# retab-dev/k-LLMs

Hardware: NVIDIA H100
Metric: consensus records/sec at n=16 (1M x 32-field); achieved HBM GB/s vs peak (higher is better)
Workload: dtype i32 codes / f64 values

## Files before the change

include/kllms_b200.h:

```cpp
#ifndef KLLMS_B200_H
#define KLLMS_B200_H

#include <stdint.h>

#ifdef __cplusplus
extern "C" {
#endif

#define KC_VERSION 200
#define KC_MAX_CANDIDATES 64

#define KC_OK 0
#define KC_EINVAL (-1)
#define KC_ECUDA (-2)
#define KC_ENODEV (-3)
#define KC_ENOMEM (-4)

#define KC_CODE_NONE (-1)
#define KC_CODE_ABSENT (-2)

#define KC_F64_NONE_BITS 0x7FF8C0DE00000000ULL
#define KC_F64_ABSENT_BITS 0x7FF8C0DF00000000ULL

#define KC_META_IDX(m) ((uint32_t)(m) & 0x3Fu)
// ... 106 lines not shown
int kc_align_json_batch(const char *const *texts, const int64_t *lens, int64_t n_records, int32_t n, double min_support_ratio, int device,
                        int32_t threads, char **out_texts, int32_t *out_status, int64_t *out_counts);
int kc_debug_similarity_json(const char *a, const char *b, double *out);
int kc_debug_alignsim(const char *const *texts, int32_t T, double *out);
int kc_debug_alignsim_nodes(const char *const *texts, const int32_t *node_len, int32_t n_nodes, int32_t lanes, int device, double *out);
int kc_debug_lsap(int32_t nr, int32_t nc, const double *cost, int32_t *row_ind, int32_t *col_ind);

int kc_consolidate_json(const char *const *texts, const int64_t *lens, int64_t n_records, int32_t n, double rel_eps,
                        double abs_eps, int device, int32_t threads, char **out_content, char **out_likelihoods,
                        uint8_t *out_status);
void kc_free_strings(char **arr, int64_t count);

#define KC_JSON_DEVICE_ONLY 1u
#define KC_JSON_NUMERIC_MEDOID 2u
#define KC_JSON_KEY_UNION 4u
#define KC_JSON_LISTS 8u
#define KC_JSON_UNICODE 16u
typedef struct kc_json_result kc_json_result;
typedef struct {
    int64_t n_records, n_device, n_host, n_python;
    int64_t input_bytes, output_bytes;
    int32_t chunks, streams;
    double h2d_ms, plan_ms , kernel_ms , emit_ms , d2h_ms;
    double device_path_wall_ms, host_path_wall_ms, wall_ms;
} kc_json_stats;
int kc_consolidate_json_packed(const char *h_text, const int64_t *h_off, int64_t n_records, int32_t n, double rel_eps, double abs_eps,
                               int device, int32_t threads, uint32_t flags, kc_json_result **out);
int kc_consolidate_json_packed_weighted(const char *h_text, const int64_t *h_off, const float *h_seq_logprob, int64_t n_records, int32_t n,
                                        double rel_eps, double abs_eps, int device, int32_t threads, uint32_t flags, kc_json_result **out);
int kc_json_result_view(kc_json_result *res, const char **text, const int64_t **content_off, const int64_t **content_len,
                        const int64_t **likelihoods_off, const int64_t **likelihoods_len, const uint8_t **status, const uint8_t **why,
                        kc_json_stats *stats);
void kc_json_result_free(kc_json_result *res);

typedef struct kc_debug_jsongpu kc_debug_jsongpu;
int kc_debug_jsongpu_plan(const char *h_text, const int64_t *h_off, int64_t n_records, int32_t n, kc_debug_jsongpu **out);
int kc_debug_jsongpu_plan_flags(const char *h_text, const int64_t *h_off, int64_t n_records, int32_t n, uint32_t flags,
                                kc_debug_jsongpu **out);
int kc_debug_jsongpu_inputs(const kc_debug_jsongpu *h, const int8_t **vote_cells, int64_t *n_vote_groups, const double **num_cells,
                            int64_t *n_num_groups, const uint8_t **status);
int kc_debug_jsongpu_emit(kc_debug_jsongpu *h, const uint32_t *vote_meta, const double *num_value, const uint32_t *num_meta,
                          const char **content, const int64_t **content_off, const char **likelihoods, const int64_t **likelihoods_off);
int kc_debug_jsongpu_group_records(const kc_debug_jsongpu *h, const int32_t **group_record);
int kc_debug_jsongpu_emit_weighted(kc_debug_jsongpu *h, const uint32_t *vote_meta, const float *vote_weight, const double *num_value,
                                   const uint32_t *num_meta, const char **content, const int64_t **content_off, const char **likelihoods,
                                   const int64_t **likelihoods_off);
int kc_debug_jsongpu_medoid_inputs(const kc_debug_jsongpu *h, const uint8_t **chars, const int32_t **str_off, const int32_t **grp_off,
                                   int64_t *n_groups);
int kc_debug_jsongpu_set_medoid(kc_debug_jsongpu *h, const int32_t *medoid_idx, const double *medoid_avg);
int kc_debug_jsongpu_set_numeric_medoid(kc_debug_jsongpu *h, const int32_t *best, const double *best_avg);
void kc_debug_jsongpu_free(kc_debug_jsongpu *h);
int kc_debug_parse_doubles(const char *text, const int64_t *off, int64_t count, double *out, uint8_t *ok);
int kc_debug_float_reprs(const double *xs, int64_t count, char *out , int32_t *lens);
int kc_debug_parse_doubles_device(const char *text, const int64_t *off, int64_t count, double *out, uint8_t *ok, int device);
int kc_debug_float_reprs_device(const double *xs, int64_t count, char *out , int32_t *lens, int device);
int kc_debug_round5(const double *xs, int64_t count, double *out);
int kc_debug_s32_texts(uint64_t seed, int64_t n_records, int32_t n, int32_t threads, char *out, int64_t cap, int64_t *off);

int32_t kc_levenshtein(const char *a, int32_t alen, const char *b, int32_t blen);

void *kc_host_alloc(uint64_t bytes);
void kc_host_free(void *p);

#ifdef __cplusplus
}
#endif
// ... 2 lines not shown
```

k_llms_b200/_native.py:

```python
from __future__ import annotations

import ctypes
import os
from typing import Optional, Tuple

_HERE = os.path.dirname(os.path.abspath(__file__))
LIB_PATH = os.environ.get("KLLMS_B200_LIB") or os.path.join(_HERE, "libkllms_b200.so")

KC_OK, KC_EINVAL, KC_ECUDA, KC_ENODEV, KC_ENOMEM = 0, -1, -2, -3, -4
MAX_CANDIDATES = 64
CODE_NONE, CODE_ABSENT = -1, -2
F64_NONE_BITS = 0x7FF8C0DE00000000
F64_ABSENT_BITS = 0x7FF8C0DF00000000
FLAG_HAS_VALUE, FLAG_SINGLE, FLAG_TIE, FLAG_NO_FINITE = 1, 2, 4, 8
OUT_LOCAL, OUT_MULTIMEM, OUT_PEERS = 0, 1, 2

_vp, _i32, _i64, _u32, _u64, _f64 = ctypes.c_void_p, ctypes.c_int32, ctypes.c_int64, ctypes.c_uint32, ctypes.c_uint64, ctypes.c_double
_int, _str, _pp = ctypes.c_int, ctypes.c_char_p, ctypes.POINTER(ctypes.c_void_p)
_CONSENSUS_HOST = [_vp, _i32, _vp, _vp, _i32, _i64, _i32, _f64, _f64, _vp, _vp, _vp, _vp, _int, _vp]

_SIGNATURES = {
    "kc_version": (_int, []),
    "kc_last_error": (_str, []),
    "kc_device_count": (_int, []),
# ... 2 lines not shown
    "kc_vote_i32": (_int, [_vp, _i64, _i32, _vp, _i32, _vp, _vp, _vp]),
    "kc_vote_i32_ex": (_int, [_vp, _i64, _i32, _vp, _i32, _vp, _vp, _u32, _vp]),
    "kc_vote_i32_peers": (_int, [_vp, _i64, _i32, _vp, _i32, _vp, _vp, _i32, _vp, _vp]),
    "kc_vote_i32_peers_packed": (_int, [_vp, _i64, _i32, _vp, _i32, _vp, _vp, _vp, _i32, _vp, _vp, _vp]),
    "kc_vote_i32_wire": (_int, [_vp, _i64, _i32, _vp, _i32, _vp, _vp, _vp, _i32, _i32, _vp, _vp, _vp]),
    "kc_vote_i8": (_int, [_vp, _i64, _i32, _vp, _i32, _vp, _vp, _vp]),
    "kc_numeric_f64": (_int, [_vp, _i64, _i32, _f64, _f64, _vp, _vp, _vp]),
    "kc_numeric_f64_ex": (_int, [_vp, _i64, _i32, _f64, _f64, _vp, _vp, _u32, _vp]),
    "kc_numeric_f64_peers": (_int, [_vp, _i64, _i32, _f64, _f64, _vp, _vp, _i32, _vp, _vp]),
    "kc_push_results": (_int, [_vp, _vp, _i64, _vp, _vp, _i64, _vp, _vp, _vp, _i32, _i32, _vp, _vp, _i32, _vp]),
    "kc_confidence_f64": (_int, [_vp, _i64, _i32, _vp, _vp, _vp]),
    "kc_logprob_sum_f32": (_int, [_vp, _vp, _i64, _vp, _vp]),
    "kc_weighted_vote_i32": (_int, [_vp, _vp, _i64, _i32, _i32, _vp, _vp, _vp, _vp, _vp]),
    "kc_weighted_vote_groups_i8": (_int, [_vp, _i64, _i32, _vp, _vp, _i64, _vp, _vp, _vp, _vp]),
    "kc_consensus_host": (_int, _CONSENSUS_HOST),
    "kc_consensus_host_i8": (_int, _CONSENSUS_HOST),
    "kc_host_alloc": (_vp, [_u64]),
    "kc_host_free": (None, [_vp]),
    "kc_medoid_str": (_int, [_vp, _vp, _vp, _i64, _i32, _vp, _vp, _vp]),
    "kc_medoid_str_method": (_int, [_vp, _vp, _vp, _i64, _i32, _i32, _vp, _vp, _vp]),
    "kc_medoid_str_host": (_int, [_vp, _i64, _vp, _vp, _i64, _i32, _vp, _vp, _int]),
    "kc_numeric_medoid_f64": (_int, [_vp, _i64, _i32, _vp, _vp, _vp]),
    "kc_levenshtein": (_int, [_str, _i32, _str, _i32]),
    "kc_consolidate_json": (_int, [_vp, _vp, _i64, _i32, _f64, _f64, _int, _i32, _vp, _vp, _vp]),
    "kc_free_strings": (None, [_vp, _i64]),
    "kc_align_json": (_int, [ctypes.POINTER(_str), _vp, _i32, _f64, ctypes.POINTER(_str)]),
    "kc_align_json_batch": (_int, [_vp, _vp, _i64, _i32, _f64, _int, _i32, _vp, _vp, _vp]),
    "kc_json_plan": (_int, [_vp, _vp, _i64, _i32, _i32, _pp]),
    "kc_json_inputs": (_int, [_vp] * 10),
    "kc_json_emit": (_int, [_vp] * 9),
    "kc_json_free": (None, [_vp]),
    "kc_consolidate_json_packed": (_int, [_vp, _vp, _i64, _i32, _f64, _f64, _int, _i32, _u32, _pp]),
    "kc_consolidate_json_packed_weighted": (_int, [_vp, _vp, _vp, _i64, _i32, _f64, _f64, _int, _i32, _u32, _pp]),
    "kc_json_result_view": (_int, [_vp] + [_pp] * 7 + [_vp]),
    "kc_json_result_free": (None, [_vp]),
    "kc_debug_similarity_json": (_int, [_str, _str, ctypes.POINTER(_f64)]),
    "kc_debug_lsap": (_int, [_i32, _i32, _vp, _vp, _vp]),
    "kc_debug_alignsim": (_int, [_vp, _i32, _vp]),
    "kc_debug_alignsim_nodes": (_int, [_vp, _vp, _i32, _i32, _int, _vp]),
    "kc_debug_jsongpu_plan": (_int, [_vp, _vp, _i64, _i32, _pp]),
    "kc_debug_jsongpu_plan_flags": (_int, [_vp, _vp, _i64, _i32, _u32, _pp]),
    "kc_debug_jsongpu_inputs": (_int, [_vp] * 6),
    "kc_debug_jsongpu_emit": (_int, [_vp, _vp, _vp, _vp] + [_pp] * 4),
    "kc_debug_jsongpu_group_records": (_int, [_vp, _pp]),
    "kc_debug_jsongpu_emit_weighted": (_int, [_vp, _vp, _vp, _vp, _vp] + [_pp] * 4),
    "kc_debug_jsongpu_medoid_inputs": (_int, [_vp] + [_pp] * 3 + [ctypes.POINTER(_i64)]),
    "kc_debug_jsongpu_set_medoid": (_int, [_vp, _vp, _vp]),
    "kc_debug_jsongpu_set_numeric_medoid": (_int, [_vp, _vp, _vp]),
    "kc_debug_jsongpu_free": (None, [_vp]),
    "kc_debug_parse_doubles": (_int, [_vp, _vp, _i64, _vp, _vp]),
    "kc_debug_float_reprs": (_int, [_vp, _i64, _vp, _vp]),
    "kc_debug_parse_doubles_device": (_int, [_vp, _vp, _i64, _vp, _vp, _int]),
    "kc_debug_float_reprs_device": (_int, [_vp, _i64, _vp, _vp, _int]),
    "kc_debug_round5": (_int, [_vp, _i64, _vp]),
    "kc_debug_s32_texts": (_int, [_u64, _i64, _i32, _i32, _vp, _i64, _vp]),
}
EXPORTS = tuple(_SIGNATURES)


class NativeError(RuntimeError):
    def __init__(self, code: int, what: str):
        super().__init__(f"libkllms_b200: {what} (code {code})")
        self.code = code


_lib: Optional[ctypes.CDLL] = None
# ... 420 lines not shown
```

k_llms_b200/csrc/kc_jsongpu.cu:

```cuda
#include <cuda_runtime.h>

#include <algorithm>
#include <atomic>
#include <chrono>
#include <cstdio>
#include <cstdlib>
#include <cstring>
#include <mutex>
#include <string>
#include <thread>
#include <type_traits>
#include <vector>

#include <cub/device/device_scan.cuh>
#include <nvtx3/nvToolsExt.h>

#include "../../include/kllms_b200.h"
#include "kc_internal.h"
#include "kc_jsongpu.cuh"

namespace {

using kc::js::Chunk;
using kc::js::Tok;

#define R_(call)                              \
    do {                                      \
        if (const int rc_ = (call)) return rc_; \
    } while (0)

enum Stage { RECORDS, SLOTS, UNION, SCRATCH, CSR, OFF };
struct Units {
    size_t R, B, T = 0, P = 0, S = 0;
};
template <class Alloc>
int chunk_arrays(const Alloc &alloc, Chunk &ch, Stage stage, const Units &u, size_t keep, bool vrec) {
    const size_t n = (size_t)ch.n;
    int k = 0;
    auto a = [&](Stage st, auto *&ptr, size_t count, size_t per, size_t plus, int fill, bool on_device) {
        const int i = k++;
        return st == stage ? alloc(i, ptr, count * per + plus, keep * per, fill, on_device) : KC_OK;
    };
    R_(a(RECORDS, ch.fcount, u.R, 1, 1, 0, true));
    R_(a(RECORDS, ch.slot, u.R, 1, 1, 0, false));
// ... 7 lines not shown
    R_(a(RECORDS, ch.mcount, u.R, 1, 1, 0, true));
    R_(a(RECORDS, ch.scount, u.R, 1, 1, 0, true));
    R_(a(RECORDS, ch.ccount, u.R, 1, 1, 0, true));
    R_(a(RECORDS, ch.len_c, u.R, 1, 1, 0, true));
    R_(a(RECORDS, ch.len_l, u.R, 1, 1, 0, true));
    R_(a(SLOTS, ch.toks, u.T, n, 1, 0, false));
    R_(a(SLOTS, ch.fdesc, u.T, 1, 1, 0, false));
    R_(a(SLOTS, ch.gpos, u.T, 1, 1, 0, false));
    R_(a(SLOTS, ch.piece_c, u.T, 1, 1, 0, false));
    R_(a(SLOTS, ch.piece_l, u.T, 1, 1, 0, false));
    R_(a(SLOTS, ch.vcells, u.T, n, 16, 0xFF, true));
    R_(a(SLOTS, ch.xcells, u.T, n, 2, 0, true));
    R_(a(vrec ? SLOTS : OFF, ch.vrec, u.T, 1, 1, 0xFF, false));
    R_(a(UNION, ch.ucand, u.P, n, 0, 0, false));
    R_(a(UNION, ch.ubase, u.P, 1, 0, 0, false));
    R_(a(UNION, ch.usize, u.P, 1, 0, 0, false));
    R_(a(SCRATCH, ch.utok, u.S, 1, 0, 0, false));
    R_(a(SCRATCH, ch.unode, u.S, 1, 0, 0, false));
    R_(a(SCRATCH, ch.umap, u.S, 1, 0, 0xFF, false));
    R_(a(CSR, ch.mchars, u.B, 1, 16, 0, false));
    R_(a(CSR, ch.mstr_off, u.T, n, 2, 0, false));
    R_(a(CSR, ch.mgrp_off, u.T, 1, 2, 0, false));
    return KC_OK;
}

void set_flags(Chunk &ch, uint32_t flags, uint8_t lists, int32_t aligned0) {
    ch.xmedoid = (flags & KC_JSON_NUMERIC_MEDOID) != 0;
    ch.key_union = (flags & KC_JSON_KEY_UNION) != 0;
    ch.unicode = (flags & KC_JSON_UNICODE) != 0;
    ch.lists = lists;
    ch.aligned0 = aligned0;
}

struct Worker {
    int device = -1;
    cudaStream_t stream = nullptr;
    cudaEvent_t ev[7] = {};
    kc::GrowBuf<kc::Mem::Device> text, off, counters, win, vmeta, xvalue, xmeta, out_c, out_l, scan_tmp, midx, mavg, seq, vweight;
    std::vector<kc::GrowBuf<kc::Mem::Device>> arrays;
    kc::GrowBuf<kc::Mem::Pinned> h_small;
    kc::GrowBuf<kc::Mem::Pinned> h_scan;
    bool busy = false;
    int init(int dev) {
        if (device == dev) return KC_OK;
        KC_CUDA_I(cudaStreamCreateWithFlags(&stream, cudaStreamNonBlocking));
        for (auto &e : ev) KC_CUDA_I(cudaEventCreate(&e));
        device = dev;
        return KC_OK;
    }
};

std::mutex g_pool_mu;
std::vector<Worker *> g_workers;

Worker *acquire_worker(int device) {
    std::lock_guard<std::mutex> lock(g_pool_mu);
    for (Worker *w : g_workers)
        if (!w->busy && w->device == device) {
            w->busy = true;
            return w;
        }
    Worker *w = new Worker;
    w->busy = true;
    g_workers.push_back(w);
    return w;
}
void release_worker(Worker *w) {
    std::lock_guard<std::mutex> lock(g_pool_mu);
    w->busy = false;
}

struct PinnedBlob {
    char *p = nullptr;
    size_t cap = 0;
};
std::vector<PinnedBlob> g_blob_pool;

PinnedBlob acquire_blob(size_t need) {
    {
// ... 48 lines not shown
        ptr = w.arrays[(size_t)k].as<E>();
        if (on_device) KC_CUDA_I(cudaMemsetAsync(ptr + keep_len, fill, (len - keep_len) * sizeof(E), w.stream));
        return KC_OK;
    };
    R_(chunk_arrays(dev, ch, stage, u, keep, weighted));
    if (stage != SLOTS) return KC_OK;
    const size_t T1 = std::max<size_t>(u.T, 1);
    R_(w.win.reserve(T1 * 4));
    R_(w.vmeta.reserve(T1 * 4));
    R_(w.xvalue.reserve(T1 * 8));
    R_(w.xmeta.reserve(T1 * 4));
    ch.vmeta = w.vmeta.as<uint32_t>();
    ch.xvalue = w.xvalue.as<double>();
    ch.xmeta = w.xmeta.as<uint32_t>();
    ch.xbest = w.xmeta.as<int32_t>();
    ch.xavg = w.xvalue.as<double>();
    if (weighted) {
        R_(w.vweight.reserve(T1 * 4));
        ch.vweight = w.vweight.as<float>();
    }
    return KC_OK;
}

template <typename T>
void exclusive_scan(T *v, size_t len) {
    T acc = 0;
    for (size_t i = 0; i < len; ++i) {
        const T c = v[i];
        v[i] = acc;
        acc += c;
    }
}

}

struct kc_json_result {
    int64_t R = 0;
    PinnedBlob blob;
    std::atomic<int64_t> used{0};
    std::vector<int64_t> c_off, c_len, l_off, l_len;
    std::vector<uint8_t> status, why;
    std::string heap;
    kc_json_stats stats{};
};

namespace {

struct ChunkStage {
    float h2d = 0, plan = 0, kernels = 0, emit = 0, d2h = 0;
};

int union_round(Worker &w, Chunk &ch, Units &u, int team, int grid, bool weighted, unsigned long long *h_cnt) {
    cudaStream_t s = w.stream;
    const int32_t P = (int32_t)u.P;
    R_(device_arrays(w, ch, UNION, u, 0, weighted));
    ch.uslot = (uint32_t)u.T;
    kc::js::union_count_kernel<<<grid, 128, 0, s>>>(ch, team, P);
    KC_CUDA_I(cudaGetLastError());
    KC_CUDA_I(cudaMemcpyAsync(h_cnt, ch.counters, 48, cudaMemcpyDeviceToHost, s));
    KC_CUDA_I(cudaStreamSynchronize(s));
    u.S = std::max<size_t>(h_cnt[4], 1);
    if (u.S >= ((size_t)1 << 32)) return kc_fail(KC_EINVAL, "kc_consolidate_json_packed: %zu union scratch entries in one chunk", u.S);
    R_(device_arrays(w, ch, SCRATCH, u, 0, weighted));
    kc::js::union_build_kernel<<<grid, 128, 0, s>>>(ch, team, P);
    KC_CUDA_I(cudaGetLastError());
    KC_CUDA_I(cudaMemcpyAsync(h_cnt, ch.counters, 48, cudaMemcpyDeviceToHost, s));
    KC_CUDA_I(cudaStreamSynchronize(s));
    if (const size_t U = h_cnt[5]) {
        const size_t keep = u.T;
        u.T += U;
        if (u.T >= ((size_t)1 << 32)) return kc_fail(KC_EINVAL, "kc_consolidate_json_packed: %zu field slots in one chunk", u.T);
        R_(device_arrays(w, ch, SLOTS, u, keep, weighted));
    }
    kc::js::union_plan_kernel<<<grid, 128, 0, s>>>(ch, team, P);
    KC_CUDA_I(cudaGetLastError());
    KC_CUDA_I(cudaMemcpyAsync(h_cnt, ch.counters, 48, cudaMemcpyDeviceToHost, s));
    KC_CUDA_I(cudaStreamSynchronize(s));
    return KC_OK;
}

int run_chunk(Worker &w, const char *h_text, const int64_t *h_off, const float *h_seq, uint32_t flags, uint8_t lists, const int64_t *dst,
              int64_t r0, int64_t r1, int32_t n, double rel_eps, double abs_eps, int sm_count, kc_json_result &res, ChunkStage &st) {
    const int64_t Rc = r1 - r0;
    const int64_t b0 = h_off[r0 * n], b1 = h_off[r1 * n];
    const size_t bytes = (size_t)(b1 - b0);
    if (bytes >= ((size_t)1 << 32)) return kc_fail(KC_EINVAL, "kc_consolidate_json_packed: chunk of %zu bytes", bytes);
    cudaStream_t s = w.stream;
    const bool weighted = h_seq != nullptr;
    Chunk ch{};
    ch.R = (int32_t)Rc;
    ch.n = n;
    set_flags(ch, flags, lists, INT32_MAX);
    Units u{(size_t)Rc, bytes};
    R_(device_arrays(w, ch, RECORDS, u, 0, weighted));
    R_(w.text.reserve(bytes + 16));
    R_(w.off.reserve((size_t)(Rc * n + 1) * 8));
    R_(w.counters.reserve(48));
    R_(w.h_small.reserve(64));
    R_(w.h_scan.reserve((size_t)(Rc + 1) * 16 + (size_t)Rc));
    if (h_seq) R_(w.seq.reserve((size_t)std::max<int64_t>(Rc * n, 1) * 4));
    size_t tmp_bytes = 0, tmp_bytes32 = 0;
    cub::DeviceScan::ExclusiveSum(nullptr, tmp_bytes, (const int64_t *)nullptr, (int64_t *)nullptr, (int)(Rc + 1), s);
    cub::DeviceScan::ExclusiveSum(nullptr, tmp_bytes32, (const uint32_t *)nullptr, (uint32_t *)nullptr, (int)(Rc + 1), s);
    R_(w.scan_tmp.reserve(std::max(tmp_bytes, tmp_bytes32) + 256));
    ch.text = w.text.as<uint8_t>();
    ch.off = w.off.as<int64_t>();
    ch.counters = w.counters.as<unsigned long long>();

    nvtxRangePushA("kc_json: H2D texts");
    KC_CUDA_I(cudaEventRecord(w.ev[0], s));
    KC_CUDA_I(cudaMemcpyAsync(w.text.p, h_text + b0, bytes, cudaMemcpyHostToDevice, s));
    KC_CUDA_I(cudaMemcpyAsync(w.off.p, h_off + r0 * n, (size_t)(Rc * n + 1) * 8, cudaMemcpyHostToDevice, s));
    if (h_seq) KC_CUDA_I(cudaMemcpyAsync(w.seq.p, h_seq + r0 * n, (size_t)(Rc * n) * 4, cudaMemcpyHostToDevice, s));
    KC_CUDA_I(cudaEventRecord(w.ev[1], s));
    nvtxRangePop();
    nvtxRangePushA("kc_json: plan (A0 count, A1 scan/type/encode)");

    const int team = team_size(n);
    const int tpw = 32 / team;
    auto grid_for = [&](int64_t threads_needed) {
        const int64_t blocks = (threads_needed + 127) / 128;
        return (int)std::max<int64_t>(1, std::min<int64_t>(blocks, (int64_t)sm_count * 16));
    };
    auto team_grid = [&](int64_t units) { return grid_for((units + tpw - 1) / tpw * 32); };
    kc::js::count_kernel<<<grid_for(Rc), 128, 0, s>>>(ch);
    KC_CUDA_I(cudaGetLastError());
    size_t tb = w.scan_tmp.cap;
    KC_CUDA_I(cub::DeviceScan::ExclusiveSum(w.scan_tmp.p, tb, (const uint32_t *)ch.fcount, ch.slot, (int)(Rc + 1), s));
    uint32_t *h_total = w.h_small.as<uint32_t>();
    KC_CUDA_I(cudaMemcpyAsync(h_total, ch.slot + Rc, 4, cudaMemcpyDeviceToHost, s));
    KC_CUDA_I(cudaStreamSynchronize(s));
    u.T = *h_total;
    R_(device_arrays(w, ch, SLOTS, u, 0, weighted));
    KC_CUDA_I(cudaMemsetAsync(w.counters.p, 0, 48, s));
    int64_t gv = 0, gx = 0, gm = 0;
    if (u.T) {
        kc::js::plan_kernel<<<team_grid(Rc), 128, 0, s>>>(ch, team);
        KC_CUDA_I(cudaGetLastError());
        unsigned long long *h_cnt = w.h_small.as<unsigned long long>() + 1;
        KC_CUDA_I(cudaMemcpyAsync(h_cnt, w.counters.p, 32, cudaMemcpyDeviceToHost, s));
        KC_CUDA_I(cudaStreamSynchronize(s));
        if ((u.P = h_cnt[3]))
            R_(union_round(w, ch, u, team, team_grid((int64_t)u.P), weighted, h_cnt));
        gv = (int64_t)h_cnt[0];
        gx = (int64_t)h_cnt[1];
        gm = (int64_t)h_cnt[2];
    }
    if (gm) {
        R_(device_arrays(w, ch, CSR, u, 0, weighted));
        R_(w.midx.reserve((u.T + 1) * 4));
        R_(w.mavg.reserve((u.T + 1) * 8));
        ch.midx = w.midx.as<int32_t>();
        ch.mavg = w.mavg.as<double>();
        for (uint32_t *cnt : {ch.mcount, ch.scount, ch.ccount}) {
            tb = w.scan_tmp.cap;
            KC_CUDA_I(cub::DeviceScan::ExclusiveSum(w.scan_tmp.p, tb, (const uint32_t *)cnt, cnt, (int)(Rc + 1), s));
        }
        kc::js::medoid_kernel<<<team_grid(Rc), 128, 0, s>>>(ch, team);
        KC_CUDA_I(cudaGetLastError());
    }
    KC_CUDA_I(cudaEventRecord(w.ev[2], s));
    nvtxRangePop();
    nvtxRangePushA("kc_json: K1 vote + K2 numeric + K4 medoid");
    if (gv && h_seq)
        R_(kc_weighted_vote_groups_i8(ch.vcells, gv, n, ch.vrec, w.seq.as<float>(), Rc, w.win.as<int32_t>(), w.vmeta.as<uint32_t>(),
                                      w.vweight.as<float>(), s));
    else if (gv)
        R_(kc_vote_i8(ch.vcells, gv, n, nullptr, 1, w.win.as<int32_t>(), w.vmeta.as<uint32_t>(), s));
    if (gx && ch.xmedoid) R_(kc_numeric_medoid_f64(ch.xcells, gx, n, w.xmeta.as<int32_t>(), w.xvalue.as<double>(), s));
    else if (gx) R_(kc_numeric_f64(ch.xcells, gx, n, rel_eps, abs_eps, w.xvalue.as<double>(), w.xmeta.as<uint32_t>(), s));
    if (gm) R_(kc_medoid_str(ch.mchars, ch.mstr_off, ch.mgrp_off, gm, std::max(2, n), w.midx.as<int32_t>(), w.mavg.as<double>(), s));
    KC_CUDA_I(cudaEventRecord(w.ev[3], s));
    nvtxRangePop();
    nvtxRangePushA("kc_json: emit (C0 lengths, C1 write)");
    kc::js::len_kernel<<<team_grid(Rc), 128, 0, s>>>(ch, team);
    KC_CUDA_I(cudaGetLastError());
    tb = w.scan_tmp.cap;
    KC_CUDA_I(cub::DeviceScan::ExclusiveSum(w.scan_tmp.p, tb, (const int64_t *)ch.len_c, ch.len_c, (int)(Rc + 1), s));
    tb = w.scan_tmp.cap;
    KC_CUDA_I(cub::DeviceScan::ExclusiveSum(w.scan_tmp.p, tb, (const int64_t *)ch.len_l, ch.len_l, (int)(Rc + 1), s));
    int64_t *h_scan_c = w.h_scan.as<int64_t>(), *h_scan_l = h_scan_c + (Rc + 1);
    uint8_t *h_status = (uint8_t *)(h_scan_l + (Rc + 1));
    KC_CUDA_I(cudaMemcpyAsync(h_scan_c, ch.len_c, (size_t)(Rc + 1) * 8, cudaMemcpyDeviceToHost, s));
    KC_CUDA_I(cudaMemcpyAsync(h_scan_l, ch.len_l, (size_t)(Rc + 1) * 8, cudaMemcpyDeviceToHost, s));
    KC_CUDA_I(cudaMemcpyAsync(h_status, ch.status, (size_t)Rc, cudaMemcpyDeviceToHost, s));
    KC_CUDA_I(cudaStreamSynchronize(s));
    const int64_t out_c_bytes = h_scan_c[Rc], out_l_bytes = h_scan_l[Rc];
    R_(w.out_c.reserve((size_t)std::max<int64_t>(out_c_bytes, 1)));
    R_(w.out_l.reserve((size_t)std::max<int64_t>(out_l_bytes, 1)));
    ch.out_c = w.out_c.as<uint8_t>();
    ch.out_l = w.out_l.as<uint8_t>();
    if (out_c_bytes) {
        kc::js::write_kernel<<<team_grid(Rc), 128, 0, s>>>(ch, team);
        KC_CUDA_I(cudaGetLastError());
    }
    KC_CUDA_I(cudaEventRecord(w.ev[4], s));
    nvtxRangePop();
    nvtxRangePushA("kc_json: D2H texts");
    const int64_t need = out_c_bytes + out_l_bytes;
    const int64_t pos = res.used.fetch_add(need);
    if (pos + need > (int64_t)res.blob.cap) {
        res.used.fetch_sub(need);
        for (int64_t i = r0; i < r1; ++i) {
            const int64_t r = dst ? dst[i] : i;
            res.status[(size_t)r] = 1;
            res.why[(size_t)r] = (uint8_t)kc::js::D_TOO_LONG;
        }
        return KC_OK;
    }
    if (out_c_bytes) KC_CUDA_I(cudaMemcpyAsync(res.blob.p + pos, ch.out_c, (size_t)out_c_bytes, cudaMemcpyDeviceToHost, s));
    if (out_l_bytes) KC_CUDA_I(cudaMemcpyAsync(res.blob.p + pos + out_c_bytes, ch.out_l, (size_t)out_l_bytes, cudaMemcpyDeviceToHost, s));
    KC_CUDA_I(cudaEventRecord(w.ev[5], s));
    KC_CUDA_I(cudaStreamSynchronize(s));
    nvtxRangePop();
    for (int64_t i = 0; i < Rc; ++i) {
        const int64_t r = dst ? dst[r0 + i] : r0 + i;
        res.status[(size_t)r] = h_status[i] ? 1 : 0;
        res.why[(size_t)r] = h_status[i];
        res.c_off[(size_t)r] = pos + h_scan_c[i];
        res.c_len[(size_t)r] = h_scan_c[i + 1] - h_scan_c[i];
        res.l_off[(size_t)r] = pos + out_c_bytes + h_scan_l[i];
        res.l_len[(size_t)r] = h_scan_l[i + 1] - h_scan_l[i];
    }
    float ms = 0;
    cudaEventElapsedTime(&ms, w.ev[0], w.ev[1]); st.h2d += ms;
    cudaEventElapsedTime(&ms, w.ev[1], w.ev[2]); st.plan += ms;
    cudaEventElapsedTime(&ms, w.ev[2], w.ev[3]); st.kernels += ms;
    cudaEventElapsedTime(&ms, w.ev[3], w.ev[4]); st.emit += ms;
    cudaEventElapsedTime(&ms, w.ev[4], w.ev[5]); st.d2h += ms;
    return KC_OK;
}

}

namespace {

void gather(const char *h_text, const int64_t *h_off, int32_t n, const std::vector<int64_t> &idx, std::vector<const char *> &texts,
            std::vector<int64_t> &lens) {
    texts.resize(idx.size() * n);
    lens.resize(idx.size() * n);
    for (size_t i = 0; i < idx.size(); ++i)
        for (int32_t c = 0; c < n; ++c) {
            const int64_t k = idx[i] * n + c;
            texts[i * n + c] = h_text + h_off[k];
            lens[i * n + c] = h_off[k + 1] - h_off[k];
        }
}

template <class Alloc>
int align_listed(const char *h_text, const int64_t *h_off, int32_t n, int device, int32_t threads, const std::vector<int64_t> &idx, const Alloc &alloc,
                 char *&blob, std::vector<int64_t> &off, std::vector<int64_t> &dst, std::vector<int64_t> &declined) {
    const int64_t L = (int64_t)idx.size();
    std::vector<const char *> texts;
    std::vector<int64_t> lens;
    gather(h_text, h_off, n, idx, texts, lens);
    std::vector<char *> out((size_t)(L * n), nullptr);
    std::vector<int32_t> st((size_t)L, 0);
    if (const int rc = kc_align_json_batch(texts.data(), lens.data(), L, n, 0.51, device, threads, out.data(), st.data(), nullptr)) {
        kc_free_strings(out.data(), L * n);
        return rc;
    }
    off.assign(1, 0);
// ... 42 lines not shown
            for (int64_t i = 0; i < M; ++i) memcpy(&seq[(size_t)(i * n)], h_seq + dst[(size_t)i] * n, (size_t)n * 4);
        }
        size_t est = 4096;
        for (int64_t i = 0; i < M; ++i) {
            const char *t = blob + off[(size_t)(i * n)];
            const int64_t len = off[(size_t)(i * n + 1)] - off[(size_t)(i * n)];
            int64_t tokens = 1;
            for (int64_t k = 0; k < len; ++k) tokens += t[k] == ',' ? 1 : (t[k] == ']' || t[k] == '}') ? 2 : 0;
            est += (size_t)(2 * len + 32 * tokens);
        }
        const size_t need = (size_t)res.used.load() + est;
        if (need > res.blob.cap) {
            PinnedBlob bigger = acquire_blob(need);
            if (!bigger.p) rc = kc_fail(KC_ENOMEM, "kc_consolidate_json_packed: cannot grow the pinned output blob to %zu bytes", need);
            else {
                memcpy(bigger.p, res.blob.p, (size_t)res.used.load());
                release_blob(res.blob);
                res.blob = bigger;
            }
        }
        if (!rc) rc = run_round(blob, off.data(), h_seq ? seq.data() : nullptr, M, (uint8_t)2, dst.data());
    }
    release_blob(texts);
    return rc;
}

}

extern "C" {

namespace {

int consolidate_packed(const char *h_text, const int64_t *h_off, const float *h_seq, int64_t n_records, int32_t n, double rel_eps,
                       double abs_eps, int device, int32_t threads, uint32_t flags, kc_json_result **out) {
    if (!out) return kc_fail(KC_EINVAL, "kc_consolidate_json_packed: NULL out");
    if (h_seq || (flags & KC_JSON_NUMERIC_MEDOID)) flags |= KC_JSON_DEVICE_ONLY;
    *out = nullptr;
    if (n < 2 || n > KC_MAX_CANDIDATES) return kc_fail(KC_EINVAL, "kc_consolidate_json_packed: n=%d outside [2,%d]", n, KC_MAX_CANDIDATES);
    if (n_records < 0 || (n_records && (!h_text || !h_off))) return kc_fail(KC_EINVAL, "kc_consolidate_json_packed: bad arguments");
    if (!(rel_eps >= 0.0) || !(abs_eps >= 0.0)) return kc_fail(KC_EINVAL, "kc_consolidate_json_packed: rel_eps/abs_eps must be >= 0");
    const auto t_start = std::chrono::steady_clock::now();
    int prev = 0;
    KC_CUDA_I(cudaGetDevice(&prev));
    KC_CUDA_I(cudaSetDevice(device));
    int sm_count = 0, cc_major = 0;
    KC_CUDA_I(cudaDeviceGetAttribute(&sm_count, cudaDevAttrMultiProcessorCount, device));
    KC_CUDA_I(cudaDeviceGetAttribute(&cc_major, cudaDevAttrComputeCapabilityMajor, device));
    if (cc_major != 9) {
        cudaSetDevice(prev);
        return kc_fail(KC_ENODEV, "device %d has compute capability %d.x; this library is sm_90a only", device, cc_major);
    }
    kc_json_result *res = new (std::nothrow) kc_json_result;
    if (!res) return kc_fail(KC_ENOMEM, "kc_consolidate_json_packed: out of memory");
    const int64_t R = n_records;
    res->R = R;
    res->c_off.assign((size_t)R, 0);
    res->c_len.assign((size_t)R, 0);
    res->l_off.assign((size_t)R, 0);
    res->l_len.assign((size_t)R, 0);
    res->status.assign((size_t)R, 1);
    res->why.assign((size_t)R, 0);
    const int64_t total_bytes = R ? h_off[R * n] - h_off[0] : 0;
    res->blob = acquire_blob((size_t)(total_bytes / n * 3 + (1 << 20)));
    if (!res->blob.p) {
        delete res;
        cudaSetDevice(prev);
        return kc_fail(KC_ENOMEM, "kc_consolidate_json_packed: cannot allocate the pinned output blob");
    }
    size_t chunk_bytes = (size_t)64 << 20;
    if (const char *e = getenv("KC_JSON_CHUNK_MB")) chunk_bytes = (size_t)std::min(1024, std::max(1, atoi(e))) << 20;
    int max_workers = 3;
    if (const char *e = getenv("KC_JSON_STREAMS")) max_workers = std::max(1, std::min(8, atoi(e)));
    int n_chunks = 0, n_streams = 0;
    std::vector<ChunkStage> stages((size_t)max_workers);
    auto run_round = [&](const char *text, const int64_t *off, const float *seq, int64_t Rb, uint8_t lists, const int64_t *dst) -> int {
        std::vector<int64_t> cuts{0};
        int64_t r = 0;
        while (r < Rb) {
            const int64_t start = off[r * n];
            int64_t lo = r + 1, hi = Rb;
            while (lo < hi) {
                const int64_t mid = lo + (hi - lo + 1) / 2;
                if ((size_t)(off[mid * n] - start) <= chunk_bytes) lo = mid;
                else hi = mid - 1;
            }
            r = lo;
            cuts.push_back(r);
        }
        const int chunks = (int)cuts.size() - 1;
        const int n_workers = std::max(1, std::min(max_workers, chunks));
        n_chunks += chunks;
        n_streams = std::max(n_streams, n_workers);
        std::vector<Worker *> workers;
        for (int i = 0; i < n_workers; ++i) workers.push_back(acquire_worker(device));
        std::vector<int> rcs((size_t)n_workers, KC_OK);
        std::vector<std::string> errs((size_t)n_workers);
        std::atomic<int> next{0};
        auto body = [&](int wi) {
            cudaSetDevice(device);
            Worker &w = *workers[(size_t)wi];
            int rc = w.init(device);
            while (!rc) {
                const int k = next.fetch_add(1);
                if (k >= chunks) break;
                rc = run_chunk(w, text, off, seq, flags, lists, dst, cuts[(size_t)k], cuts[(size_t)k + 1], n, rel_eps, abs_eps, sm_count, *res,
                               stages[(size_t)wi]);
            }
            if (rc) {
                cudaStreamSynchronize(w.stream);
                errs[(size_t)wi] = kc_last_error();
            }
            rcs[(size_t)wi] = rc;
        };
        if (n_workers == 1) {
            body(0);
        } else {
            std::vector<std::thread> pool;
            for (int i = 0; i < n_workers; ++i) pool.emplace_back(body, i);
            for (auto &t : pool) t.join();
        }
        for (Worker *w : workers) release_worker(w);
        for (int i = 0; i < n_workers; ++i)
            if (rcs[(size_t)i]) return kc_fail(rcs[(size_t)i], "%s", errs[(size_t)i].c_str());
        return KC_OK;
    };
    const bool lists = (flags & KC_JSON_LISTS) != 0;
    int rc = run_round(h_text, h_off, h_seq, R, lists ? 1 : 0, nullptr);
    if (!rc && lists) rc = list_round(*res, h_text, h_off, h_seq, n, device, threads, run_round);
    const auto t_gpu = std::chrono::steady_clock::now();
    int64_t n_declined = 0, n_host = 0;
    if (!rc) {
        std::vector<int64_t> idx;
        for (int64_t r = 0; r < R; ++r) {
            if (!res->status[(size_t)r]) continue;
            ++n_declined;
            if (res->why[(size_t)r] != kc::js::D_ALIGN) idx.push_back(r);
        }
        if (!idx.empty() && !(flags & KC_JSON_DEVICE_ONLY)) {
            const int64_t D = (int64_t)idx.size();
            std::vector<const char *> texts;
            std::vector<int64_t> lens;
            gather(h_text, h_off, n, idx, texts, lens);
            std::vector<char *> oc((size_t)D, nullptr), ol((size_t)D, nullptr);
            std::vector<uint8_t> hs((size_t)D, 1);
            rc = kc_consolidate_json(texts.data(), lens.data(), D, n, rel_eps, abs_eps, device, threads, oc.data(), ol.data(), hs.data());
            if (!rc) {
                int64_t pos = res->used.load(), extra = 0;
                for (int64_t i = 0; i < D; ++i)
                    if (hs[(size_t)i] == 0) extra += (int64_t)(strlen(oc[(size_t)i]) + strlen(ol[(size_t)i]));
                char *base = res->blob.p;
                if (pos + extra > (int64_t)res->blob.cap) {
                    res->heap.resize((size_t)(pos + extra));
                    memcpy(&res->heap[0], res->blob.p, (size_t)pos);
                    release_blob(res->blob);
                    res->blob = PinnedBlob{};
                    base = &res->heap[0];
                }
                for (int64_t i = 0; i < D; ++i) {
                    if (hs[(size_t)i] != 0) continue;
                    const int64_t r = idx[(size_t)i];
                    const size_t lc = strlen(oc[(size_t)i]), ll = strlen(ol[(size_t)i]);
                    memcpy(base + pos, oc[(size_t)i], lc);
// ... 25 lines not shown
    s.n_device = R - n_declined;
    s.n_host = n_host;
    s.n_python = n_declined - n_host;
    s.input_bytes = total_bytes;
    s.output_bytes = res->used.load();
    s.chunks = n_chunks;
    s.streams = n_streams;
    for (auto &g : stages) {
        s.h2d_ms += g.h2d;
        s.plan_ms += g.plan;
        s.kernel_ms += g.kernels;
        s.emit_ms += g.emit;
        s.d2h_ms += g.d2h;
    }
    s.device_path_wall_ms = ms(t_start, t_gpu);
    s.host_path_wall_ms = ms(t_gpu, t_end);
    s.wall_ms = ms(t_start, t_end);
    *out = res;
    return KC_OK;
}

}

int kc_consolidate_json_packed(const char *h_text, const int64_t *h_off, int64_t n_records, int32_t n, double rel_eps, double abs_eps,
                               int device, int32_t threads, uint32_t flags, kc_json_result **out) {
    return consolidate_packed(h_text, h_off, nullptr, n_records, n, rel_eps, abs_eps, device, threads, flags, out);
}

int kc_consolidate_json_packed_weighted(const char *h_text, const int64_t *h_off, const float *h_seq_logprob, int64_t n_records, int32_t n,
                                        double rel_eps, double abs_eps, int device, int32_t threads, uint32_t flags, kc_json_result **out) {
    if (n_records > 0 && !h_seq_logprob) return kc_fail(KC_EINVAL, "kc_consolidate_json_packed_weighted: NULL h_seq_logprob");
    static const float none = 0.0f;
    return consolidate_packed(h_text, h_off, h_seq_logprob ? h_seq_logprob : &none, n_records, n, rel_eps, abs_eps, device, threads, flags, out);
}

int kc_json_result_view(kc_json_result *res, const char **text, const int64_t **content_off, const int64_t **content_len,
                        const int64_t **likelihoods_off, const int64_t **likelihoods_len, const uint8_t **status, const uint8_t **why,
                        kc_json_stats *stats) {
    if (!res) return kc_fail(KC_EINVAL, "kc_json_result_view: NULL result");
    if (text) *text = res->blob.p ? res->blob.p : res->heap.data();
    if (content_off) *content_off = res->c_off.data();
    if (content_len) *content_len = res->c_len.data();
    if (likelihoods_off) *likelihoods_off = res->l_off.data();
    if (likelihoods_len) *likelihoods_len = res->l_len.data();
    if (status) *status = res->status.data();
    if (why) *why = res->why.data();
    if (stats) *stats = res->stats;
    return KC_OK;
}

void kc_json_result_free(kc_json_result *res) {
    if (!res) return;
    release_blob(res->blob);
    delete res;
}


struct kc_debug_jsongpu {
    std::vector<int64_t> off;
    std::vector<uint8_t> text;
    int32_t n = 0;
    int64_t R = 0;
    std::vector<std::vector<uint8_t>> arrays;
    unsigned long long counters[6] = {0, 0, 0, 0, 0, 0};
    std::vector<uint8_t> out_c, out_l;
    int64_t R_out = 0;
// ... 410 lines not shown
```

Baseline: 1.021 billion.

## Double-buffer chunk uploads on a copy stream and skip result zero-init

Each worker gets a dedicated copy stream and two input buffer sets, so the next chunk's text and offsets upload while the current chunk runs its kernels. Offsets and weights are staged through pinned memory. Result vectors now use a no-init allocator to avoid zero-filling large arrays, with the too-long path explicitly zeroing its entries. The change also adds an optional timeline trace and a debug entry point that takes texts already on the device. In exchange it holds extra device and pinned buffers and adds cross-stream event synchronisation.

After: 1.019 billion, median of 6. Within noise of the previous version (-0.3%).

```diff
diff --git a/include/kllms_b200.h b/include/kllms_b200.h
--- a/include/kllms_b200.h
+++ b/include/kllms_b200.h
@@ -162,6 +162,8 @@
                         const int64_t **likelihoods_off, const int64_t **likelihoods_len, const uint8_t **status, const uint8_t **why,
                         kc_json_stats *stats);
 void kc_json_result_free(kc_json_result *res);
+int kc_debug_jsongpu_device_texts(const char *d_text, const int64_t *h_off, int64_t n_records, int32_t n, int device, uint32_t flags,
+                                  kc_json_result **out);
 
 typedef struct kc_debug_jsongpu kc_debug_jsongpu;
 int kc_debug_jsongpu_plan(const char *h_text, const int64_t *h_off, int64_t n_records, int32_t n, kc_debug_jsongpu **out);
diff --git a/k_llms_b200/_native.py b/k_llms_b200/_native.py
--- a/k_llms_b200/_native.py
+++ b/k_llms_b200/_native.py
@@ -58,6 +58,7 @@
     "kc_json_free": (None, [_vp]),
     "kc_consolidate_json_packed": (_int, [_vp, _vp, _i64, _i32, _f64, _f64, _int, _i32, _u32, _pp]),
     "kc_consolidate_json_packed_weighted": (_int, [_vp, _vp, _vp, _i64, _i32, _f64, _f64, _int, _i32, _u32, _pp]),
+    "kc_debug_jsongpu_device_texts": (_int, [_vp, _vp, _i64, _i32, _int, _u32, _pp]),
     "kc_json_result_view": (_int, [_vp] + [_pp] * 7 + [_vp]),
     "kc_json_result_free": (None, [_vp]),
     "kc_debug_similarity_json": (_int, [_str, _str, ctypes.POINTER(_f64)]),
diff --git a/k_llms_b200/csrc/kc_jsongpu.cu b/k_llms_b200/csrc/kc_jsongpu.cu
--- a/k_llms_b200/csrc/kc_jsongpu.cu
+++ b/k_llms_b200/csrc/kc_jsongpu.cu
@@ -6,10 +6,12 @@
 #include <cstdio>
 #include <cstdlib>
 #include <cstring>
+#include <memory>
 #include <mutex>
 #include <string>
 #include <thread>
 #include <type_traits>
+#include <utility>
 #include <vector>
 
 #include <cub/device/device_scan.cuh>
@@ -83,19 +85,32 @@
     ch.aligned0 = aligned0;
 }
 
+struct Inputs {
+    kc::GrowBuf<kc::Mem::Device> text, off, seq;
+    kc::GrowBuf<kc::Mem::Pinned> staged;
+    cudaEvent_t started = nullptr, copied = nullptr;
+};
+
 struct Worker {
     int device = -1;
-    cudaStream_t stream = nullptr;
+    cudaStream_t stream = nullptr, copy = nullptr;
     cudaEvent_t ev[7] = {};
-    kc::GrowBuf<kc::Mem::Device> text, off, counters, win, vmeta, xvalue, xmeta, out_c, out_l, scan_tmp, midx, mavg, seq, vweight;
+    Inputs in[2];
+    kc::GrowBuf<kc::Mem::Device> counters, win, vmeta, xvalue, xmeta, out_c, out_l, scan_tmp, midx, mavg, vweight;
     std::vector<kc::GrowBuf<kc::Mem::Device>> arrays;
     kc::GrowBuf<kc::Mem::Pinned> h_small;
     kc::GrowBuf<kc::Mem::Pinned> h_scan;
     bool busy = false;
+    int index = 0;
     int init(int dev) {
         if (device == dev) return KC_OK;
         KC_CUDA_I(cudaStreamCreateWithFlags(&stream, cudaStreamNonBlocking));
+        KC_CUDA_I(cudaStreamCreateWithFlags(&copy, cudaStreamNonBlocking));
         for (auto &e : ev) KC_CUDA_I(cudaEventCreate(&e));
+        for (Inputs &i : in) {
+            KC_CUDA_I(cudaEventCreate(&i.started));
+            KC_CUDA_I(cudaEventCreate(&i.copied));
+        }
         device = dev;
         return KC_OK;
     }
@@ -210,14 +225,30 @@
     }
 }
 
+template <typename T>
+struct NoInit : std::allocator<T> {
+    template <typename U>
+    struct rebind {
+        using other = NoInit<U>;
+    };
+    template <typename U>
+    void construct(U *p) noexcept {
+        ::new ((void *)p) U;
+    }
+    template <typename U, typename... A>
+    void construct(U *p, A &&...a) {
+        ::new ((void *)p) U(std::forward<A>(a)...);
+    }
+};
+
 }
 
 struct kc_json_result {
     int64_t R = 0;
     PinnedBlob blob;
     std::atomic<int64_t> used{0};
-    std::vector<int64_t> c_off, c_len, l_off, l_len;
-    std::vector<uint8_t> status, why;
+    std::vector<int64_t, NoInit<int64_t>> c_off, c_len, l_off, l_len;
+    std::vector<uint8_t, NoInit<uint8_t>> status, why;
     std::string heap;
     kc_json_stats stats{};
 };
@@ -228,7 +259,29 @@
     float h2d = 0, plan = 0, kernels = 0, emit = 0, d2h = 0;
 };
 
-int union_round(Worker &w, Chunk &ch, Units &u, int team, int grid, bool weighted, unsigned long long *h_cnt) {
+struct Timeline {
+    cudaEvent_t origin = nullptr;
+    std::chrono::steady_clock::time_point t0;
+    std::mutex mu;
+    std::string lines;
+};
+
+int wait_for(cudaStream_t s, Timeline *tl, std::string &waits, const char *what) {
+    if (!tl) {
+        KC_CUDA_I(cudaStreamSynchronize(s));
+        return KC_OK;
+    }
+    const auto a = std::chrono::steady_clock::now();
+    KC_CUDA_I(cudaStreamSynchronize(s));
+    const auto b = std::chrono::steady_clock::now();
+    char buf[128];
+    snprintf(buf, sizeof buf, "%s[\"%s\", %.4f, %.4f]", waits.empty() ? "" : ", ", what,
+             std::chrono::duration<double, std::milli>(a - tl->t0).count(), std::chrono::duration<double, std::milli>(b - a).count());
+    waits += buf;
+    return KC_OK;
+}
+
+int union_round(Worker &w, Chunk &ch, Units &u, int team, int grid, bool weighted, unsigned long long *h_cnt, Timeline *tl, std::string &waits) {
     cudaStream_t s = w.stream;
     const int32_t P = (int32_t)u.P;
     R_(device_arrays(w, ch, UNION, u, 0, weighted));
@@ -236,14 +289,14 @@
     kc::js::union_count_kernel<<<grid, 128, 0, s>>>(ch, team, P);
     KC_CUDA_I(cudaGetLastError());
     KC_CUDA_I(cudaMemcpyAsync(h_cnt, ch.counters, 48, cudaMemcpyDeviceToHost, s));
-    KC_CUDA_I(cudaStreamSynchronize(s));
+    R_(wait_for(s, tl, waits, "union scratch"));
     u.S = std::max<size_t>(h_cnt[4], 1);
     if (u.S >= ((size_t)1 << 32)) return kc_fail(KC_EINVAL, "kc_consolidate_json_packed: %zu union scratch entries in one chunk", u.S);
     R_(device_arrays(w, ch, SCRATCH, u, 0, weighted));
     kc::js::union_build_kernel<<<grid, 128, 0, s>>>(ch, team, P);
     KC_CUDA_I(cudaGetLastError());
     KC_CUDA_I(cudaMemcpyAsync(h_cnt, ch.counters, 48, cudaMemcpyDeviceToHost, s));
-    KC_CUDA_I(cudaStreamSynchronize(s));
+    R_(wait_for(s, tl, waits, "union rows"));
     if (const size_t U = h_cnt[5]) {
         const size_t keep = u.T;
         u.T += U;
@@ -253,16 +306,37 @@
     kc::js::union_plan_kernel<<<grid, 128, 0, s>>>(ch, team, P);
     KC_CUDA_I(cudaGetLastError());
     KC_CUDA_I(cudaMemcpyAsync(h_cnt, ch.counters, 48, cudaMemcpyDeviceToHost, s));
-    KC_CUDA_I(cudaStreamSynchronize(s));
-    return KC_OK;
-}
-
-int run_chunk(Worker &w, const char *h_text, const int64_t *h_off, const float *h_seq, uint32_t flags, uint8_t lists, const int64_t *dst,
-              int64_t r0, int64_t r1, int32_t n, double rel_eps, double abs_eps, int sm_count, kc_json_result &res, ChunkStage &st) {
+    R_(wait_for(s, tl, waits, "union counters"));
+    return KC_OK;
+}
+
+int upload(Worker &w, Inputs &in, const char *h_text, const int64_t *h_off, const float *h_seq, int64_t r0, int64_t r1, int32_t n,
+           bool device_text) {
+    const int64_t b0 = h_off[r0 * n];
+    const size_t bytes = (size_t)(h_off[r1 * n] - b0);
+    if (bytes >= ((size_t)1 << 32)) return kc_fail(KC_EINVAL, "kc_consolidate_json_packed: chunk of %zu bytes", bytes);
+    const size_t off_bytes = (size_t)((r1 - r0) * n + 1) * 8, seq_bytes = h_seq ? (size_t)((r1 - r0) * n) * 4 : 0;
+    if (!device_text) R_(in.text.reserve(bytes + 16));
+    R_(in.off.reserve(off_bytes));
+    if (h_seq) R_(in.seq.reserve(std::max<size_t>(seq_bytes, 4)));
+    R_(in.staged.reserve(off_bytes + seq_bytes));
+    memcpy(in.staged.p, h_off + r0 * n, off_bytes);
+    if (h_seq) memcpy(in.staged.as<char>() + off_bytes, h_seq + r0 * n, seq_bytes);
+    cudaStream_t c = w.copy;
+    KC_CUDA_I(cudaEventRecord(in.started, c));
+    if (!device_text) KC_CUDA_I(cudaMemcpyAsync(in.text.p, h_text + b0, bytes, cudaMemcpyHostToDevice, c));
+    KC_CUDA_I(cudaMemcpyAsync(in.off.p, in.staged.p, off_bytes, cudaMemcpyHostToDevice, c));
+    if (h_seq) KC_CUDA_I(cudaMemcpyAsync(in.seq.p, in.staged.as<char>() + off_bytes, seq_bytes, cudaMemcpyHostToDevice, c));
+    KC_CUDA_I(cudaEventRecord(in.copied, c));
+    return KC_OK;
+}
+
+int run_chunk(Worker &w, Inputs &in, const char *h_text, const int64_t *h_off, const float *h_seq, uint32_t flags, uint8_t lists,
+              const int64_t *dst, int64_t r0, int64_t r1, int32_t n, double rel_eps, double abs_eps, int sm_count, kc_json_result &res,
+              ChunkStage &st, bool device_text, Timeline *tl) {
     const int64_t Rc = r1 - r0;
     const int64_t b0 = h_off[r0 * n], b1 = h_off[r1 * n];
     const size_t bytes = (size_t)(b1 - b0);
-    if (bytes >= ((size_t)1 << 32)) return kc_fail(KC_EINVAL, "kc_consolidate_json_packed: chunk of %zu bytes", bytes);
     cudaStream_t s = w.stream;
     const bool weighted = h_seq != nullptr;
     Chunk ch{};
@@ -271,27 +345,20 @@
     set_flags(ch, flags, lists, INT32_MAX);
     Units u{(size_t)Rc, bytes};
     R_(device_arrays(w, ch, RECORDS, u, 0, weighted));
-    R_(w.text.reserve(bytes + 16));
-    R_(w.off.reserve((size_t)(Rc * n + 1) * 8));
     R_(w.counters.reserve(48));
     R_(w.h_small.reserve(64));
     R_(w.h_scan.reserve((size_t)(Rc + 1) * 16 + (size_t)Rc));
-    if (h_seq) R_(w.seq.reserve((size_t)std::max<int64_t>(Rc * n, 1) * 4));
     size_t tmp_bytes = 0, tmp_bytes32 = 0;
     cub::DeviceScan::ExclusiveSum(nullptr, tmp_bytes, (const int64_t *)nullptr, (int64_t *)nullptr, (int)(Rc + 1), s);
     cub::DeviceScan::ExclusiveSum(nullptr, tmp_bytes32, (const uint32_t *)nullptr, (uint32_t *)nullptr, (int)(Rc + 1), s);
     R_(w.scan_tmp.reserve(std::max(tmp_bytes, tmp_bytes32) + 256));
-    ch.text = w.text.as<uint8_t>();
-    ch.off = w.off.as<int64_t>();
+    ch.text = device_text ? (const uint8_t *)h_text + b0 : in.text.as<uint8_t>();
+    ch.off = in.off.as<int64_t>();
     ch.counters = w.counters.as<unsigned long long>();
-
-    nvtxRangePushA("kc_json: H2D texts");
-    KC_CUDA_I(cudaEventRecord(w.ev[0], s));
-    KC_CUDA_I(cudaMemcpyAsync(w.text.p, h_text + b0, bytes, cudaMemcpyHostToDevice, s));
-    KC_CUDA_I(cudaMemcpyAsync(w.off.p, h_off + r0 * n, (size_t)(Rc * n + 1) * 8, cudaMemcpyHostToDevice, s));
-    if (h_seq) KC_CUDA_I(cudaMemcpyAsync(w.seq.p, h_seq + r0 * n, (size_t)(Rc * n) * 4, cudaMemcpyHostToDevice, s));
+    std::string waits;
+
+    KC_CUDA_I(cudaStreamWaitEvent(s, in.copied, 0));
     KC_CUDA_I(cudaEventRecord(w.ev[1], s));
-    nvtxRangePop();
     nvtxRangePushA("kc_json: plan (A0 count, A1 scan/type/encode)");
 
     const int team = team_size(n);
@@ -307,7 +374,7 @@
     KC_CUDA_I(cub::DeviceScan::ExclusiveSum(w.scan_tmp.p, tb, (const uint32_t *)ch.fcount, ch.slot, (int)(Rc + 1), s));
     uint32_t *h_total = w.h_small.as<uint32_t>();
     KC_CUDA_I(cudaMemcpyAsync(h_total, ch.slot + Rc, 4, cudaMemcpyDeviceToHost, s));
-    KC_CUDA_I(cudaStreamSynchronize(s));
+    R_(wait_for(s, tl, waits, "slot total"));
     u.T = *h_total;
     R_(device_arrays(w, ch, SLOTS, u, 0, weighted));
     KC_CUDA_I(cudaMemsetAsync(w.counters.p, 0, 48, s));
@@ -317,9 +384,9 @@
         KC_CUDA_I(cudaGetLastError());
         unsigned long long *h_cnt = w.h_small.as<unsigned long long>() + 1;
         KC_CUDA_I(cudaMemcpyAsync(h_cnt, w.counters.p, 32, cudaMemcpyDeviceToHost, s));
-        KC_CUDA_I(cudaStreamSynchronize(s));
+        R_(wait_for(s, tl, waits, "counters"));
         if ((u.P = h_cnt[3]))
-            R_(union_round(w, ch, u, team, team_grid((int64_t)u.P), weighted, h_cnt));
+            R_(union_round(w, ch, u, team, team_grid((int64_t)u.P), weighted, h_cnt, tl, waits));
         gv = (int64_t)h_cnt[0];
         gx = (int64_t)h_cnt[1];
         gm = (int64_t)h_cnt[2];
@@ -341,7 +408,7 @@
     nvtxRangePop();
     nvtxRangePushA("kc_json: K1 vote + K2 numeric + K4 medoid");
     if (gv && h_seq)
-        R_(kc_weighted_vote_groups_i8(ch.vcells, gv, n, ch.vrec, w.seq.as<float>(), Rc, w.win.as<int32_t>(), w.vmeta.as<uint32_t>(),
+        R_(kc_weighted_vote_groups_i8(ch.vcells, gv, n, ch.vrec, in.seq.as<float>(), Rc, w.win.as<int32_t>(), w.vmeta.as<uint32_t>(),
                                       w.vweight.as<float>(), s));
     else if (gv)
         R_(kc_vote_i8(ch.vcells, gv, n, nullptr, 1, w.win.as<int32_t>(), w.vmeta.as<uint32_t>(), s));
@@ -362,7 +429,7 @@
     KC_CUDA_I(cudaMemcpyAsync(h_scan_c, ch.len_c, (size_t)(Rc + 1) * 8, cudaMemcpyDeviceToHost, s));
     KC_CUDA_I(cudaMemcpyAsync(h_scan_l, ch.len_l, (size_t)(Rc + 1) * 8, cudaMemcpyDeviceToHost, s));
     KC_CUDA_I(cudaMemcpyAsync(h_status, ch.status, (size_t)Rc, cudaMemcpyDeviceToHost, s));
-    KC_CUDA_I(cudaStreamSynchronize(s));
+    R_(wait_for(s, tl, waits, "lengths"));
     const int64_t out_c_bytes = h_scan_c[Rc], out_l_bytes = h_scan_l[Rc];
     R_(w.out_c.reserve((size_t)std::max<int64_t>(out_c_bytes, 1)));
     R_(w.out_l.reserve((size_t)std::max<int64_t>(out_l_bytes, 1)));
@@ -383,13 +450,15 @@
             const int64_t r = dst ? dst[i] : i;
             res.status[(size_t)r] = 1;
             res.why[(size_t)r] = (uint8_t)kc::js::D_TOO_LONG;
-        }
+            res.c_off[(size_t)r] = res.c_len[(size_t)r] = res.l_off[(size_t)r] = res.l_len[(size_t)r] = 0;
+        }
+        KC_CUDA_I(cudaStreamSynchronize(s));
         return KC_OK;
     }
     if (out_c_bytes) KC_CUDA_I(cudaMemcpyAsync(res.blob.p + pos, ch.out_c, (size_t)out_c_bytes, cudaMemcpyDeviceToHost, s));
     if (out_l_bytes) KC_CUDA_I(cudaMemcpyAsync(res.blob.p + pos + out_c_bytes, ch.out_l, (size_t)out_l_bytes, cudaMemcpyDeviceToHost, s));
     KC_CUDA_I(cudaEventRecord(w.ev[5], s));
-    KC_CUDA_I(cudaStreamSynchronize(s));
+    R_(wait_for(s, tl, waits, "d2h"));
     nvtxRangePop();
     for (int64_t i = 0; i < Rc; ++i) {
         const int64_t r = dst ? dst[r0 + i] : r0 + i;
@@ -401,11 +470,26 @@
         res.l_len[(size_t)r] = h_scan_l[i + 1] - h_scan_l[i];
     }
     float ms = 0;
-    cudaEventElapsedTime(&ms, w.ev[0], w.ev[1]); st.h2d += ms;
+    cudaEventElapsedTime(&ms, in.started, in.copied); st.h2d += ms;
     cudaEventElapsedTime(&ms, w.ev[1], w.ev[2]); st.plan += ms;
     cudaEventElapsedTime(&ms, w.ev[2], w.ev[3]); st.kernels += ms;
     cudaEventElapsedTime(&ms, w.ev[3], w.ev[4]); st.emit += ms;
     cudaEventElapsedTime(&ms, w.ev[4], w.ev[5]); st.d2h += ms;
+    if (tl) {
+        float t[7];
+        cudaEventElapsedTime(&t[0], tl->origin, in.started);
+        cudaEventElapsedTime(&t[1], tl->origin, in.copied);
+        for (int i = 1; i < 6; ++i) cudaEventElapsedTime(&t[i + 1], tl->origin, w.ev[i]);
+        char buf[512];
+        snprintf(buf, sizeof buf,
+                 "{\"stream\": %d, \"r0\": %lld, \"r1\": %lld, \"bytes\": %zu, \"h2d\": [%.4f, %.4f], \"plan\": [%.4f, %.4f], "
+                 "\"kernels\": [%.4f, %.4f], \"emit\": [%.4f, %.4f], \"d2h\": [%.4f, %.4f], \"waits\": [",
+                 w.index, (long long)r0, (long long)r1, bytes, t[0], t[1], t[2], t[3], t[3], t[4], t[4], t[5], t[5], t[6]);
+        std::lock_guard<std::mutex> lock(tl->mu);
+        tl->lines += buf;
+        tl->lines += waits;
+        tl->lines += "]}\n";
+    }
     return KC_OK;
 }
 
@@ -514,7 +598,7 @@
 namespace {
 
 int consolidate_packed(const char *h_text, const int64_t *h_off, const float *h_seq, int64_t n_records, int32_t n, double rel_eps,
-                       double abs_eps, int device, int32_t threads, uint32_t flags, kc_json_result **out) {
+                       double abs_eps, int device, int32_t threads, uint32_t flags, kc_json_result **out, bool device_text = false) {
     if (!out) return kc_fail(KC_EINVAL, "kc_consolidate_json_packed: NULL out");
     if (h_seq || (flags & KC_JSON_NUMERIC_MEDOID)) flags |= KC_JSON_DEVICE_ONLY;
     *out = nullptr;
@@ -536,12 +620,9 @@
     if (!res) return kc_fail(KC_ENOMEM, "kc_consolidate_json_packed: out of memory");
     const int64_t R = n_records;
     res->R = R;
-    res->c_off.assign((size_t)R, 0);
-    res->c_len.assign((size_t)R, 0);
-    res->l_off.assign((size_t)R, 0);
-    res->l_len.assign((size_t)R, 0);
-    res->status.assign((size_t)R, 1);
-    res->why.assign((size_t)R, 0);
+    for (auto *v : {&res->c_off, &res->c_len, &res->l_off, &res->l_len}) v->resize((size_t)R);
+    res->status.resize((size_t)R);
+    res->why.resize((size_t)R);
     const int64_t total_bytes = R ? h_off[R * n] - h_off[0] : 0;
     res->blob = acquire_blob((size_t)(total_bytes / n * 3 + (1 << 20)));
     if (!res->blob.p) {
@@ -555,6 +636,13 @@
     if (const char *e = getenv("KC_JSON_STREAMS")) max_workers = std::max(1, std::min(8, atoi(e)));
     int n_chunks = 0, n_streams = 0;
     std::vector<ChunkStage> stages((size_t)max_workers);
+    const char *tl_path = getenv("KC_JSON_TIMELINE");
+    Timeline timeline, *tl = nullptr;
+    if (tl_path && *tl_path && cudaEventCreate(&timeline.origin) == cudaSuccess) {
+        tl = &timeline;
+        tl->t0 = std::chrono::steady_clock::now();
+        cudaEventRecord(tl->origin, 0);
+    }
     auto run_round = [&](const char *text, const int64_t *off, const float *seq, int64_t Rb, uint8_t lists, const int64_t *dst) -> int {
         std::vector<int64_t> cuts{0};
         int64_t r = 0;
@@ -581,14 +669,21 @@
         auto body = [&](int wi) {
             cudaSetDevice(device);
             Worker &w = *workers[(size_t)wi];
+            w.index = wi;
             int rc = w.init(device);
-            while (!rc) {
-                const int k = next.fetch_add(1);
-                if (k >= chunks) break;
-                rc = run_chunk(w, text, off, seq, flags, lists, dst, cuts[(size_t)k], cuts[(size_t)k + 1], n, rel_eps, abs_eps, sm_count, *res,
-                               stages[(size_t)wi]);
+            int k = next.fetch_add(1), i = 0;
+            if (!rc && k < chunks) rc = upload(w, w.in[0], text, off, seq, cuts[(size_t)k], cuts[(size_t)k + 1], n, device_text);
+            while (!rc && k < chunks) {
+                const int k2 = next.fetch_add(1);
+                if (k2 < chunks) rc = upload(w, w.in[i ^ 1], text, off, seq, cuts[(size_t)k2], cuts[(size_t)k2 + 1], n, device_text);
+                if (!rc)
+                    rc = run_chunk(w, w.in[i], text, off, seq, flags, lists, dst, cuts[(size_t)k], cuts[(size_t)k + 1], n, rel_eps, abs_eps,
+                                   sm_count, *res, stages[(size_t)wi], device_text, tl);
+                k = k2;
+                i ^= 1;
             }
             if (rc) {
+                cudaStreamSynchronize(w.copy);
                 cudaStreamSynchronize(w.stream);
                 errs[(size_t)wi] = kc_last_error();
             }
@@ -610,6 +705,16 @@
     int rc = run_round(h_text, h_off, h_seq, R, lists ? 1 : 0, nullptr);
     if (!rc && lists) rc = list_round(*res, h_text, h_off, h_seq, n, device, threads, run_round);
     const auto t_gpu = std::chrono::steady_clock::now();
+    if (tl) {
+        if (FILE *f = fopen(tl_path, "a")) {
+            fprintf(f, "{\"call\": {\"records\": %lld, \"n\": %d, \"device_path_wall_ms\": %.4f, \"setup_ms\": %.4f}}\n", (long long)R, n,
+                    std::chrono::duration<double, std::milli>(t_gpu - t_start).count(),
+                    std::chrono::duration<double, std::milli>(tl->t0 - t_start).count());
+            fputs(tl->lines.c_str(), f);
+            fclose(f);
+        }
+        cudaEventDestroy(tl->origin);
+    }
     int64_t n_declined = 0, n_host = 0;
     if (!rc) {
         std::vector<int64_t> idx;
@@ -701,6 +806,12 @@
     if (n_records > 0 && !h_seq_logprob) return kc_fail(KC_EINVAL, "kc_consolidate_json_packed_weighted: NULL h_seq_logprob");
     static const float none = 0.0f;
     return consolidate_packed(h_text, h_off, h_seq_logprob ? h_seq_logprob : &none, n_records, n, rel_eps, abs_eps, device, threads, flags, out);
+}
+
+int kc_debug_jsongpu_device_texts(const char *d_text, const int64_t *h_off, int64_t n_records, int32_t n, int device, uint32_t flags,
+                                  kc_json_result **out) {
+    if (flags & KC_JSON_LISTS) return kc_fail(KC_EINVAL, "kc_debug_jsongpu_device_texts: the list round aligns host texts");
+    return consolidate_packed(d_text, h_off, nullptr, n_records, n, 0.03, 1e-6, device, 0, flags | KC_JSON_DEVICE_ONLY, out, true);
 }
 
 int kc_json_result_view(kc_json_result *res, const char **text, const int64_t **content_off, const int64_t **content_len,
```
